# KerkDovan/univer-ocr

Measured on AMD Instinct MI355X. Metric: document-images/sec (fwd+bwd) on 256x512 synthetic pages, higher is better.
Workload: dtype f32; 1 GPU; BASELINE configs[2]: my_model train step (fwd+loss+bwd+L2+SGD) of Monochrome+Paragraph+Line on (32,256,512,1) pages and Char on (32,32,64,1) line strips per GPU; batch_per_gpu=32, global_batch=32, optimizer=sgd, parallelism=dp1, h2d_inclusive=False, input_grads=True, hip_graphs=True, pipelined_lanes=True, hw_queues=4

## Files before the change

univer-ocr_amd/csrc/conv_fast.hip:

```cpp
#include "finish_group.h"
#include "conv_dims.h"

namespace {

template <int C, typename TA>
__device__ __forceinline__ void load_vec(const TA* __restrict__ p, float (&v)[C]) {
    if constexpr (C == 1) {
        v[0] = ld1(p);
    } else if constexpr (C == 2) {
        const float2 t = ld2(p);
        v[0] = t.x;
        v[1] = t.y;
    } else {
        static_assert(C % 4 == 0, "channel count must be 1, 2 or a multiple of 4");
#pragma unroll
        for (int q = 0; q < C / 4; ++q) {
            const float4 t = ld4(p + 4 * q);
            v[4 * q] = t.x;
            v[4 * q + 1] = t.y;
            v[4 * q + 2] = t.z;
            v[4 * q + 3] = t.w;
        }
    }
}
// ... 740 lines not shown
                if constexpr (CIN == 1 && PX % 4 == 0) {
                    constexpr int PWC = KW / 2, OFFS = (4 - PWC % 4) % 4;
                    if (d.pw == PWC && d.w % 4 == 0) {
                        load_row_c1<NXV, OFFS>(xb + (size_t)iyc * d.w, ix0 - OFFS, d.w, row_ok, pad, xv);
                        vec_done = true;
                    }
                }
                if (!vec_done) {
#pragma unroll
                    for (int j = 0; j < NXV; ++j) {
                        const int ix = ix0 + j;
                        if constexpr (CLAMP) {
                            load_vec<CIN>(xb + ((size_t)iyc * d.w + min(max(ix, 0), d.w - 1)) * CIN, xv[j]);
                            if (!(row_ok && ix >= 0 && ix < d.w)) {
#pragma unroll
                                for (int c = 0; c < CIN; ++c) xv[j][c] = pad;
                            }
                        } else {
                            if (row_ok && ix >= 0 && ix < d.w) {
                                load_vec<CIN>(xb + ((size_t)iy * d.w + ix) * CIN, xv[j]);
                            } else {
#pragma unroll
                                for (int c = 0; c < CIN; ++c) xv[j][c] = pad;
                            }
                        }
                    }
                }
#pragma unroll
                for (int kx = 0; kx < KW; ++kx)
#pragma unroll
                    for (int c = 0; c < CIN; ++c)
#pragma unroll
                        for (int o = 0; o < COB; ++o)
#pragma unroll
                            for (int p = 0; p < PX; ++p)
                                acc[((kyl * KW + kx) * CIN + c) * COB + o] += xv[p * SW + kx][c] * g[p][o];
            }
        }
    }
    lane_reduce_scatter<C::NP>(acc, lane);
    int base = 0;
#pragma unroll
    for (int s = 0; s < 6; ++s)
        if (lane & (32 >> s)) base += C::NP >> (s + 1);
#pragma unroll
    for (int r = 0; r < C::NP / 64; ++r) red[wv][base + r] = acc[r];
    __syncthreads();
    const int tid = wv * 64 + lane;
    float* out = partial + ((size_t)blockIdx.y * gridDim.x + blockIdx.x) * C::NP;
    for (int a = tid; a < C::NP; a += 256) out[a] = red[0][a] + red[1][a] + red[2][a] + red[3][a];
}

template <int KH, int KW, int CIN, int COUT, int KYR, int COB, int NW, int NP>
__global__ __launch_bounds__(256) void conv_wgrad_fast_finish(const float* __restrict__ partial, float* __restrict__ dw,
                                                              float* __restrict__ db, int nblocks, int use_bias,
                                                              int accumulate, float unscale) {
    __shared__ double smem[16];
    const int a = blockIdx.x, grp = blockIdx.y;
    constexpr int OCG = COUT / COB;
    const int kyg = grp / OCG, ocg = grp % OCG;
    const float* src = partial + (size_t)grp * nblocks * NP + a;
    double s = 0.0;
    for (int i = threadIdx.x; i < nblocks; i += blockDim.x) s += (double)src[(size_t)i * NP];
    s = block_reduce_sum(s, smem);
    if (threadIdx.x != 0) return;
    float* dst;
    if (a < NW) {
        const int o = a % COB, t = a / COB;
        const int c = t % CIN, tap = t / CIN;
        const int kx = tap % KW, kyl = tap / KW;
        dst = dw + (((size_t)(kyg * KYR + kyl) * KW + kx) * CIN + c) * COUT + ocg * COB + o;
    } else {
        if (kyg != 0) return;
        dst = db + ocg * COB + (a - NW);
        if (!use_bias) s = 0.0;
    }
    s *= (double)unscale;
    *dst = accumulate ? (float)((double)*dst + s) : (float)s;
}

namespace t542 {
constexpr int TH = 16, TW = 64, WH = TH + 4, WW = TW + 4, NW = 40, NB = 2, NACC = NW + NB, NP = 64;
__device__ __forceinline__ int swz(int row, int c) { return row * WW + (c & 3) * (WW / 4) + (c >> 2); }
struct Taprows {
    static constexpr int TH = t542::TH, TW = t542::TW, NW = t542::NW, NB = t542::NB, ROW = NACC;
};
}

template <typename TA>
__global__ __launch_bounds__(320) void conv_wgrad_t542(const TA* __restrict__ x, const TA* __restrict__ dy,
                                                       float* __restrict__ partial, int h, int wd, float pad,
                                                       int tiles_per_block) {
    using namespace t542;
    __shared__ float4 xs[WH * WW];
    __shared__ float2 gs[TH * TW];
    const int tid = threadIdx.x, lane = tid & 63, ky = tid >> 6;
    const int x0 = blockIdx.x * TW, b = blockIdx.z;
    const int tile0 = blockIdx.y * tiles_per_block, tiles_y = (h + TH - 1) / TH;
    const TA* xb = x + (size_t)b * h * wd * 4;
    const TA* gb = dy + (size_t)b * h * wd * 2;
    float acc[NP];
#pragma unroll
    for (int a = 0; a < NP; ++a) acc[a] = 0.f;
    const int cg = lane & 15, rsub = lane >> 4;
    const int t_end = min(tiles_y, tile0 + tiles_per_block);
    for (int t = tile0; t < t_end; ++t) {
        const int y0 = t * TH;
        __syncthreads();
        for (int e = tid; e < WH * WW; e += 320) {
            const int r = e / WW, c = e - r * WW;
            const int gy = y0 - 2 + r, gx = x0 - 2 + c;
            float4 v = ld4(xb + ((size_t)min(max(gy, 0), h - 1) * wd + min(max(gx, 0), wd - 1)) * 4);
            if (gy < 0 || gy >= h || gx < 0 || gx >= wd) v = make_float4(pad, pad, pad, pad);
            xs[swz(r, c)] = v;
        }
        for (int e = tid; e < TH * TW; e += 320) {
            const int r = e / TW, c = e - r * TW;
            const int gy = y0 + r, gx = x0 + c;
            float2 v = ld2(gb + ((size_t)min(gy, h - 1) * wd + min(gx, wd - 1)) * 2);
            if (gy >= h || gx >= wd) v = make_float2(0.f, 0.f);
            gs[e] = v;
        }
        __syncthreads();
#pragma unroll 1
        for (int it = 0; it < TH / 4; ++it) {
            const int r = it * 4 + rsub;
            float g[4][2];
            {
                const float4* gp = reinterpret_cast<const float4*>(gs + r * TW + 4 * cg);
                const float4 g01 = gp[0], g23 = gp[1];
                g[0][0] = g01.x, g[0][1] = g01.y, g[1][0] = g01.z, g[1][1] = g01.w;
                g[2][0] = g23.x, g[2][1] = g23.y, g[3][0] = g23.z, g[3][1] = g23.w;
            }
            float xv[8][4];
#pragma unroll
            for (int j = 0; j < 8; ++j) {
                const float4 v = xs[swz(r + ky, 4 * cg + j)];
                xv[j][0] = v.x, xv[j][1] = v.y, xv[j][2] = v.z, xv[j][3] = v.w;
            }
#pragma unroll
            for (int kx = 0; kx < 5; ++kx)
#pragma unroll
                for (int ci = 0; ci < 4; ++ci)
#pragma unroll
                    for (int co = 0; co < 2; ++co)
#pragma unroll
                        for (int px = 0; px < 4; ++px) acc[(kx * 4 + ci) * 2 + co] += xv[px + kx][ci] * g[px][co];
            if (ky == 0) {
#pragma unroll
                for (int px = 0; px < 4; ++px) {
                    acc[40] += g[px][0];
                    acc[41] += g[px][1];
                }
            }
        }
    }
    lane_reduce_scatter<NP>(acc, lane);
    const size_t blk = ((size_t)blockIdx.z * gridDim.y + blockIdx.y) * gridDim.x + blockIdx.x;
    if (lane < NACC) partial[(blk * 5 + ky) * NACC + lane] = acc[0];
}

template <int CIN, int COUT>
struct S2Cfg {
    static constexpr int TH = 8, TW = 32, WH = 2 * TH + 3, WW = 2 * TW + 3;
    static constexpr int NW = 5 * CIN * COUT, NACC = NW + COUT;
    static constexpr int NP = ((NACC + 63) / 64) * 64;
    static constexpr int NB = COUT, ROW = NP;
};

template <int CIN, int COUT, typename TA>
__global__ __launch_bounds__(320) void conv_wgrad_s2_tiled(const TA* __restrict__ x, const TA* __restrict__ dy,
                                                           float* __restrict__ partial, int h, int wd, int oh, int ow,
                                                           float pad, int tiles_per_block) {
    using C = S2Cfg<CIN, COUT>;
    __shared__ __attribute__((aligned(16))) float xs[C::WH * C::WW * CIN];
    __shared__ float gs[C::TH * C::TW * COUT];
    const int tid = threadIdx.x, lane = tid & 63, ky = tid >> 6;
    const int ox0 = blockIdx.x * C::TW, b = blockIdx.z;
    const int tile0 = blockIdx.y * tiles_per_block, tiles_y = (oh + C::TH - 1) / C::TH;
    const TA* xb = x + (size_t)b * h * wd * CIN;
    const TA* gb = dy + (size_t)b * oh * ow * COUT;
    float acc[C::NP];
#pragma unroll
    for (int a = 0; a < C::NP; ++a) acc[a] = 0.f;
    const int t_end = min(tiles_y, tile0 + tiles_per_block);
    for (int t = tile0; t < t_end; ++t) {
        const int oy0 = t * C::TH;
        __syncthreads();
        if constexpr (sizeof(TA) == 4 && (CIN == 1 || CIN == 4)) {
            using VX = std::conditional_t<CIN == 1, float, float4>;
            stage_batched<C::WH * C::WW, 320, 4, VX>(
                tid,
                [&](int e, bool& inside) {
                    const int r = e / C::WW, c = e - r * C::WW;
                    const int gy = 2 * oy0 - 2 + r, gx = 2 * ox0 - 2 + c;
                    inside = gy >= 0 && gy < h && gx >= 0 && gx < wd;
                    return reinterpret_cast<const VX*>(xb + ((size_t)min(max(gy, 0), h - 1) * wd + min(max(gx, 0), wd - 1)) * CIN);
                },
                [&](int e, VX v, bool inside) {
                    if constexpr (CIN == 1) xs[e] = inside ? v : pad;
                    else *reinterpret_cast<float4*>(xs + e * 4) = inside ? v : make_float4(pad, pad, pad, pad);
                });
        } else {
        for (int e = tid; e < C::WH * C::WW; e += 320) {
            const int r = e / C::WW, c = e - r * C::WW;
            const int gy = 2 * oy0 - 2 + r, gx = 2 * ox0 - 2 + c;
            float v[CIN];
            load_vec<CIN>(xb + ((size_t)min(max(gy, 0), h - 1) * wd + min(max(gx, 0), wd - 1)) * CIN, v);
            const bool in = gy >= 0 && gy < h && gx >= 0 && gx < wd;
#pragma unroll
            for (int ci = 0; ci < CIN; ++ci) xs[e * CIN + ci] = in ? v[ci] : pad;
        }
        }
        for (int e = tid; e < C::TH * C::TW; e += 320) {
            const int r = e / C::TW, c = e - r * C::TW;
            const int gy = oy0 + r, gx = ox0 + c;
            float v[COUT];
            load_vec<COUT>(gb + ((size_t)min(gy, oh - 1) * ow + min(gx, ow - 1)) * COUT, v);
            const bool in = gy < oh && gx < ow;
#pragma unroll
            for (int co = 0; co < COUT; ++co) gs[e * COUT + co] = in ? v[co] : 0.f;
        }
        __syncthreads();
#pragma unroll 1
        for (int it = 0; it < C::TH * C::TW / 64; ++it) {
            const int e = it * 64 + lane, r = e / C::TW, c = e - r * C::TW;
            float g[COUT];
#pragma unroll
            for (int co = 0; co < COUT; ++co) g[co] = gs[e * COUT + co];
            const float* xr = xs + ((2 * r + ky) * C::WW + 2 * c) * CIN;
#pragma unroll
            for (int kx = 0; kx < 5; ++kx)
#pragma unroll
                for (int ci = 0; ci < CIN; ++ci) {
                    const float xv = xr[kx * CIN + ci];
#pragma unroll
                    for (int co = 0; co < COUT; ++co) acc[(kx * CIN + ci) * COUT + co] += xv * g[co];
                }
            if (ky == 0) {
#pragma unroll
                for (int co = 0; co < COUT; ++co) acc[C::NW + co] += g[co];
            }
// ... 213 lines not shown
}

int uocr_conv_dgrad_fast(uocr_ctx* ctx, int dtype, const void* dy, const void* w, void* dx, const ConvDims& d,
                         const ActMask& mask) {
    const bool f32 = UOCR_DTYPE_BASE(dtype) == UOCR_F32;
    const C16Args c16{dy, w, nullptr, dx, 0.f, 0, UOCR_ACT_NONE, 0.f, mask};
    if (f32 && is_c16_same(d, 16, 1))
        return launch_c16(ctx, conv_c16_expand<3, 3, 2, true>, 2, c16, d, 1, UOCR_CONV_C16_EXPAND);
    if (f32 && is_c16_same(d, 1, 16))
        return launch_c16(ctx, conv_c16_reduce<3, 3, 4, true>, 4, c16, d, 1, UOCR_CONV_C16_REDUCE);
    if (f32 && d.kh == 5 && d.kw == 3 && d.sh == 2 && d.sw == 1 && d.ph == 0 && d.pw == 1 && d.cin == 1 && d.cout == 64 &&
        d.h <= 65535 && d.n <= 65535) {
        hipLaunchKernelGGL(conv_dgrad_c64s2, dim3((unsigned)((d.w + 15) / 16), d.h, d.n), dim3(256), 0, ctx->stream,
                           (const float*)dy, (const float*)w, (float*)dx, d.n, d.h, d.w, d.oh, d.ow,
                           (const float*)mask.y, mask.act, (float)mask.alpha);
        UOCR_LAUNCH_CHECK(ctx);
        uocr_note_conv(ctx, 1, UOCR_CONV_DGRAD_C64S2);
        return UOCR_OK;
    }
    if (is_5x5_s2_pad2(d) && ((d.cin == 1 && (d.cout == 1 || d.cout == 4)) || (d.cin == 4 && d.cout == 4))) {
        const dim3 grid(((d.w + 1) / 2 + 63) / 64, ((d.h + 1) / 2 + 3) / 4, d.n), block(64, 4);
        const FastDims fd{d.n, d.h, d.w, d.oh, d.ow, d.ph, d.pw};
        const int rc = uocr_act_tags<1>(ctx, UOCR_ACT_NONE, mask.act, [&](auto kinds) -> int {
            using K = decltype(kinds);
            using D = ActKinds<UOCR_ACT_DYN, UOCR_ACT_DYN>;
            UOCR_DISPATCH_TA(ctx, dtype, {
                auto launch = [&](auto kernel) {
                    hipLaunchKernelGGL(kernel, grid, block, 0, ctx->stream, (const TA*)dy, (const float*)w, (TA*)dx, fd,
                                       (const TA*)mask.y, mask.act, (float)mask.alpha);
                };
                if (d.cin == 4) launch(conv_dgrad_s2<4, 4, TA, K>);
                else if (d.cout == 1) launch(conv_dgrad_s2<1, 1, TA, D>);
                else launch(conv_dgrad_s2<1, 4, TA, D>);
            });
            UOCR_LAUNCH_CHECK(ctx);
            return UOCR_OK;
        });
        if (rc != UOCR_OK) return rc;
        uocr_note_conv(ctx, 1, UOCR_CONV_DGRAD_S2);
        return UOCR_OK;
    }
    int rc = UOCR_OK;
    if (with_fast_conv(d, [&](auto fc) { rc = uocr_noted_conv(ctx, 1, fc.DX_KERNEL, fc.dgrad(ctx, dtype, dy, w, dx, d, mask)); }))
        return rc;
    UOCR_FAIL(ctx, UOCR_ERR_UNSUPPORTED, "no fast conv kernel for this shape");
}

int uocr_conv_wgrad_fast(uocr_ctx* ctx, int dtype, const void* x, const void* dy, void* dw, void* db,
                         const ConvDims& d, double pad_value, int use_bias, int accumulate) {
    const bool f32 = UOCR_DTYPE_BASE(dtype) == UOCR_F32;
    if (f32 && is_c16_same(d, 16, 1) && pad_value == 0.0) {
        constexpr int NA = 3 * 3 * 4 + 1;
        const long budget = uocr_budget(ctx, 2048);
        int rows = (int)((d.n * d.h + budget - 1) / budget);
        rows = ((rows + 3) / 4) * 4;
        if (rows > d.h) rows = ((d.h + 3) / 4) * 4;
        const int nbands = (d.h + rows - 1) / rows, nblocks = nbands * d.n;
        uocr_note_split(ctx, nblocks, (long long)((d.h + 3) / 4) * d.n);
        int rc = uocr_need_workspace(ctx, (size_t)nblocks * 4 * NA * sizeof(float));
        if (rc) return rc;
        float* partial = (float*)ctx->workspace;
        hipLaunchKernelGGL((conv_c16_wgrad<3, 3>), dim3(nblocks), dim3(64, 4), 0, ctx->stream, (const float*)x,
                           (const float*)dy, partial, d.h, d.w, d.ph, d.pw, rows, nbands);
        UOCR_LAUNCH_CHECK(ctx);
        hipLaunchKernelGGL((conv_c16_wgrad_finish<3, 3>), dim3(NA, 4), dim3(256), 0, ctx->stream,
                           (const float*)partial, (float*)dw, (float*)db, nblocks, use_bias, accumulate);
        UOCR_LAUNCH_CHECK(ctx);
        uocr_note_conv(ctx, 2, UOCR_CONV_C16_WGRAD);
        return UOCR_OK;
    }
    if (is_5x5_s2_pad2(d) && ctx->opt_tiled == 1 && d.cin == 1 && d.cout == 4)
        return launch_wgrad_taprows<S2Cfg<1, 4>>(
            ctx, dtype, UOCR_CONV_WGRAD_S2_TILED, d.n, d.oh, d.ow, dw, db, use_bias, accumulate,
            [&](auto ta, dim3 grid, float* partial, int per_block) {
                using TA = decltype(ta);
                hipLaunchKernelGGL((conv_wgrad_s2_tiled<1, 4, TA>), grid, dim3(320), 0, ctx->stream, (const TA*)x,
                                   (const TA*)dy, partial, d.h, d.w, d.oh, d.ow, (float)pad_value, per_block);
            });
    if (is_5x5_s1_pad2(d) && d.cin == 4 && d.cout == 2)
        return launch_wgrad_taprows<t542::Taprows>(
            ctx, dtype, UOCR_CONV_WGRAD_T542, d.n, d.h, d.w, dw, db, use_bias, accumulate,
            [&](auto ta, dim3 grid, float* partial, int per_block) {
                using TA = decltype(ta);
                hipLaunchKernelGGL((conv_wgrad_t542<TA>), grid, dim3(320), 0, ctx->stream, (const TA*)x, (const TA*)dy,
                                   partial, d.h, d.w, (float)pad_value, per_block);
            });
    int rc = UOCR_OK;
    if (with_fast_conv(d, [&](auto fc) {
            rc = uocr_noted_conv(ctx, 2, UOCR_CONV_TABLE_FAST, fc.wgrad(ctx, dtype, x, dy, dw, db, d, pad_value, use_bias, accumulate));
        }))
        return rc;
    UOCR_FAIL(ctx, UOCR_ERR_UNSUPPORTED, "no fast conv kernel for this shape");
}
```

univer-ocr_amd/csrc/ctx.hip:

```cpp
#include <cstdlib>

#include "finish_group.h"
#include "gemm.h"
#include "uocr_common.h"

extern "C" {

int uocr_abi_version(void) { return UOCR_ABI_VERSION; }

int uocr_ctx_create(int device, size_t workspace_bytes, uocr_ctx** out) {
    if (!out || device < 0) return UOCR_ERR_ARG;
    *out = nullptr;
    int count = 0;
    if (hipGetDeviceCount(&count) != hipSuccess || device >= count) return UOCR_ERR_HIP;
    if (hipSetDevice(device) != hipSuccess) return UOCR_ERR_HIP;
    uocr_ctx* ctx = new uocr_ctx();
    ctx->device = device;
#ifdef UOCR_EXPERIMENTS
    if (const char* e = getenv("UOCR_H3")) ctx->opt_h3 = atoi(e);
#endif
    if (const char* e = getenv("UOCR_PAIR_PF")) ctx->opt_pair_pf = atoi(e);
    if (const char* e = getenv("UOCR_WGRAD_BANDS")) ctx->opt_wgrad_bands = atoi(e);
    if (hipStreamCreateWithFlags(&ctx->stream, hipStreamNonBlocking) != hipSuccess) {
        delete ctx;
// ... 8 lines not shown
            return UOCR_ERR_HIP;
        }
        ctx->workspace_bytes = workspace_bytes;
    }
    if (hipMalloc((void**)&ctx->sync, UOCR_SYNC_WORDS * sizeof(unsigned)) != hipSuccess ||
        hipMemsetAsync(ctx->sync, 0, UOCR_SYNC_WORDS * sizeof(unsigned), ctx->stream) != hipSuccess ||
        hipStreamSynchronize(ctx->stream) != hipSuccess) {
        if (ctx->sync) hipFree(ctx->sync);
        if (ctx->workspace) hipFree(ctx->workspace);
        hipStreamDestroy(ctx->stream);
        delete ctx;
        return UOCR_ERR_HIP;
    }
    *out = ctx;
    return UOCR_OK;
}

int uocr_ctx_create_cu_mask(int device, size_t workspace_bytes, const uint32_t* cu_mask, int mask_words, uocr_ctx** out) {
    if (!out || !cu_mask || mask_words <= 0) return UOCR_ERR_ARG;
    int rc = uocr_ctx_create(device, workspace_bytes, out);
    if (rc != UOCR_OK) return rc;
    uocr_ctx* ctx = *out;
    hipStream_t masked = nullptr;
    if (hipExtStreamCreateWithCUMask(&masked, (uint32_t)mask_words, cu_mask) != hipSuccess) {
        uocr_ctx_destroy(ctx);
        *out = nullptr;
        return UOCR_ERR_HIP;
    }
    hipStreamDestroy(ctx->stream);
    ctx->stream = masked;
    int cus = 0;
    for (int i = 0; i < mask_words; ++i) cus += __builtin_popcount(cu_mask[i]);
    if (cus > 0 && cus < ctx->cu_count) ctx->cu_count = cus;
    return UOCR_OK;
}

int uocr_ctx_destroy(uocr_ctx* ctx) {
    UOCR_CHECK_CTX(ctx);
    hipSetDevice(ctx->device);
    hipStreamSynchronize(ctx->stream);
    if (ctx->workspace) hipFree(ctx->workspace);
    if (ctx->sync) hipFree(ctx->sync);
    uocr_gemm_defer_free(ctx);
    uocr_finish_defer_free(ctx);
    if (ctx->owns_stream) hipStreamDestroy(ctx->stream);
    delete ctx;
    return UOCR_OK;
}

int uocr_ctx_set_stream(uocr_ctx* ctx, void* hip_stream) {
    UOCR_CHECK_CTX(ctx);
    if (ctx->owns_stream) {
        UOCR_HIP(ctx, hipStreamSynchronize(ctx->stream));
        UOCR_HIP(ctx, hipStreamDestroy(ctx->stream));
        ctx->owns_stream = false;
    }
    ctx->stream = (hipStream_t)hip_stream;
    return UOCR_OK;
}

int uocr_ctx_set_option(uocr_ctx* ctx, const char* key, int value) {
    UOCR_CHECK_CTX(ctx);
    UOCR_REQUIRE(ctx, key != nullptr);
    if (!strcmp(key, "mfma")) ctx->opt_mfma = value;
    else if (!strcmp(key, "fast_paths")) ctx->opt_fast = value;
    else if (!strcmp(key, "tiled")) ctx->opt_tiled = value;
    else if (!strcmp(key, "split_blocks")) ctx->opt_split = value;
    else if (!strcmp(key, "split_min")) ctx->opt_split_min = value;
    else if (!strcmp(key, "gemm_bm")) ctx->opt_bm = value;
    else if (!strcmp(key, "xcd_remap")) ctx->opt_xcd = value;
    else if (!strcmp(key, "h16")) ctx->opt_h16 = value;
    else if (!strcmp(key, "t32")) {
        if (value & ~UOCR_T32_BUILT)
            UOCR_FAIL(ctx, UOCR_ERR_UNSUPPORTED, "option t32 = %d asks for kernels this library was built without "
                      "(UOCR_BUILD_EXPERIMENTS=1 ./build.sh)", value);
        ctx->opt_t32 = value;
    }
    else if (!strcmp(key, "pair_band")) ctx->opt_pair_band = value;
    else if (!strcmp(key, "pair_g")) ctx->opt_pair_g = value;
    else if (!strcmp(key, "group_blocks")) ctx->opt_group_blocks = value;
    else if (!strcmp(key, "wgrad_bands") && value >= 0) ctx->opt_wgrad_bands = value;
    else if (!strcmp(key, "max_blocks") && value >= 0) ctx->opt_max_blocks = value;
    else if (!strcmp(key, "act_dispatch")) ctx->opt_act_dispatch = value != 0;
    else if (!strcmp(key, "h3")) {
#ifndef UOCR_EXPERIMENTS
        if (value) UOCR_FAIL(ctx, UOCR_ERR_UNSUPPORTED, "option h3: this library was built without conv_h3 "
                             "(UOCR_BUILD_EXPERIMENTS=1 ./build.sh)");
#endif
        ctx->opt_h3 = value;
    }
    else if (!strcmp(key, "pair_pf")) ctx->opt_pair_pf = value;
    else UOCR_FAIL(ctx, UOCR_ERR_ARG, "unknown option '%s'", key);
    return UOCR_OK;
}

int uocr_ctx_last_split(uocr_ctx* ctx, int* blocks, long long* items) {
    return uocr_report_read(ctx, UOCR_REPORT_SPLIT, blocks, items);
}

int uocr_ctx_last_gemm(uocr_ctx* ctx, int* bm, int* gm, int* gn, int* nsplit) {
    return uocr_report_read(ctx, UOCR_REPORT_GEMM, bm, gm, gn, nsplit);
}

int uocr_ctx_last_gemm_group(uocr_ctx* ctx, int* problems, int* split_problems) {
    return uocr_report_read(ctx, UOCR_REPORT_GEMM_GROUP, problems, split_problems);
}

int uocr_ctx_last_pair(uocr_ctx* ctx, int* kernel, int* g, int* mode, int* pf, int* nw, int* blocks_x, int* bands,
                       int* band_h) {
    return uocr_report_read(ctx, UOCR_REPORT_PAIR, kernel, g, mode, pf, nw, blocks_x, bands, band_h);
}

int uocr_ctx_last_conv(uocr_ctx* ctx, int* entry, int* kernel) {
    return uocr_report_read(ctx, UOCR_REPORT_CONV, entry, kernel);
}

void* uocr_ctx_get_stream(uocr_ctx* ctx) { return ctx ? (void*)ctx->stream : nullptr; }

int uocr_ctx_reserve_workspace(uocr_ctx* ctx, size_t bytes) {
    UOCR_CHECK_CTX(ctx);
    if (bytes <= ctx->workspace_bytes) return UOCR_OK;
    UOCR_HIP(ctx, hipSetDevice(ctx->device));
    UOCR_HIP(ctx, hipStreamSynchronize(ctx->stream));
    if (ctx->workspace) UOCR_HIP(ctx, hipFree(ctx->workspace));
    ctx->workspace = nullptr;
    ctx->workspace_bytes = 0;
    UOCR_HIP(ctx, hipMalloc(&ctx->workspace, bytes));
    ctx->workspace_bytes = bytes;
    return UOCR_OK;
}

const char* uocr_last_error(uocr_ctx* ctx) { return ctx ? ctx->err : "null context"; }

int uocr_malloc(uocr_ctx* ctx, size_t bytes, void** out) {
    UOCR_CHECK_CTX(ctx);
    UOCR_REQUIRE(ctx, out != nullptr);
    UOCR_HIP(ctx, hipSetDevice(ctx->device));
    UOCR_HIP(ctx, hipMalloc(out, bytes ? bytes : 1));
    return UOCR_OK;
}

int uocr_free(uocr_ctx* ctx, void* ptr) {
    UOCR_CHECK_CTX(ctx);
    if (ptr) UOCR_HIP(ctx, hipFree(ptr));
    return UOCR_OK;
}

int uocr_memset_zero(uocr_ctx* ctx, void* ptr, size_t bytes) {
    UOCR_CHECK_CTX(ctx);
    if (!bytes) return UOCR_OK;
    UOCR_REQUIRE(ctx, ptr != nullptr);
    UOCR_HIP(ctx, hipMemsetAsync(ptr, 0, bytes, ctx->stream));
    return UOCR_OK;
}

int uocr_h2d(uocr_ctx* ctx, void* dst, const void* src_host, size_t bytes) {
    UOCR_CHECK_CTX(ctx);
    if (!bytes) return UOCR_OK;
    UOCR_REQUIRE(ctx, dst && src_host);
    UOCR_HIP(ctx, hipMemcpyAsync(dst, src_host, bytes, hipMemcpyHostToDevice, ctx->stream));
    return UOCR_OK;
}

int uocr_d2h_sync(uocr_ctx* ctx, void* dst_host, const void* src, size_t bytes) {
    UOCR_CHECK_CTX(ctx);
    if (!bytes) return UOCR_OK;
// ... 106 lines not shown
```

univer-ocr_amd/csrc/uocr_common.h:

```cpp
#pragma once
#include <hip/hip_runtime.h>
#include <stdint.h>
#include <stdio.h>
#include <string.h>

#include <type_traits>

#include "univer_hip.h"

enum uocr_report_id {
    UOCR_REPORT_SPLIT,
    UOCR_REPORT_GEMM,
    UOCR_REPORT_GEMM_GROUP,
    UOCR_REPORT_PAIR,
    UOCR_REPORT_CONV,
    UOCR_REPORT_LABEL,
    UOCR_REPORT_LABEL_BATCH,
    UOCR_REPORT_CHAR_LABEL,
    UOCR_REPORT_LINE_CROP,
    UOCR_REPORT_ROTATE,
    UOCR_REPORT_ROTATION_SEARCH,
    UOCR_REPORT_PRED_TO_TEXT,
    UOCR_REPORT_PACK_LINES,
    UOCR_REPORT_COUNT
};
constexpr int UOCR_REPORT_VALUES = 8;

struct uocr_ctx {
    int device = 0;
    hipStream_t stream = nullptr;
    bool owns_stream = true;
    void* workspace = nullptr;
    size_t workspace_bytes = 0;
    const double* snap_src = nullptr;
    int snap_count = 0;
    double* snap_ring = nullptr;
    int snap_ring_len = 0;
    unsigned* snap_counter = nullptr;
    void* gemm_defer = nullptr;
    void* finish_defer = nullptr;
    unsigned* sync = nullptr;
    int cu_count = 256;
    int opt_mfma = 1;
    int opt_fast = 1;
    int opt_tiled = 1;
    int opt_split = 1024;
    int opt_split_min = 3;
    int opt_xcd = 1;
    int opt_bm = 0;
    int opt_h16 = 1;
    int opt_t32 = 2;
    int opt_pair_band = 0;
    int opt_pair_pf = -1;
    int opt_h3 = 0;
    int opt_group_blocks = 0;
    int opt_wgrad_bands = 0;
    int opt_pair_g = 4;
    int opt_act_dispatch = 1;
    int opt_max_blocks = 0;
    long long report[UOCR_REPORT_COUNT][UOCR_REPORT_VALUES] = {};
    char err[512] = {};
};

constexpr int UOCR_SYNC_WORDS = 1 << 18;
#ifdef UOCR_EXPERIMENTS
constexpr int UOCR_T32_BUILT = 255;
#else
constexpr int UOCR_T32_BUILT = 2;
#endif

#define UOCR_FAIL(ctx, code, ...)                                   \
    do {                                                            \
        if (ctx) snprintf((ctx)->err, sizeof((ctx)->err), __VA_ARGS__); \
        return (code);                                              \
    } while (0)

#define UOCR_HIP(ctx, call)                                                              \
    do {                                                                                 \
        hipError_t e_ = (call);                                                          \
        if (e_ != hipSuccess)                                                            \
            UOCR_FAIL(ctx, UOCR_ERR_HIP, "%s failed: %s (%s:%d)", #call, hipGetErrorString(e_), \
                      __FILE__, __LINE__);                                               \
    } while (0)

#define UOCR_LAUNCH_CHECK(ctx)                                                           \
    do {                                                                                 \
        hipError_t e_ = hipGetLastError();                                               \
        if (e_ != hipSuccess)                                                            \
            UOCR_FAIL(ctx, UOCR_ERR_HIP, "kernel launch failed: %s (%s:%d)", hipGetErrorString(e_), \
                      __FILE__, __LINE__);                                               \
    } while (0)

#define UOCR_REQUIRE(ctx, cond)                                                          \
    do {                                                                                 \
        if (!(cond)) UOCR_FAIL(ctx, UOCR_ERR_ARG, "bad argument: %s (%s:%d)", #cond, __FILE__, __LINE__); \
    } while (0)

#define UOCR_CHECK_CTX(ctx) \
    do {                    \
        if (!(ctx)) return UOCR_ERR_ARG; \
    } while (0)

template <typename... V>
static inline void uocr_note(uocr_ctx* ctx, uocr_report_id id, V... v) {
    static_assert(sizeof...(V) >= 1 && sizeof...(V) <= UOCR_REPORT_VALUES, "a report holds 1 to UOCR_REPORT_VALUES values");
    long long* slot = ctx->report[id];
    ((*slot++ = (long long)v), ...);
}
template <typename... T>
static inline int uocr_report_read(uocr_ctx* ctx, uocr_report_id id, T*... out) {
    static_assert(sizeof...(T) >= 1 && sizeof...(T) <= UOCR_REPORT_VALUES, "a report holds 1 to UOCR_REPORT_VALUES values");
    UOCR_CHECK_CTX(ctx);
    if (!(out && ...)) UOCR_FAIL(ctx, UOCR_ERR_ARG, "bad argument: null out pointer of launch report %d", (int)id);
    const long long* slot = ctx->report[id];
    ((*out = (T)*slot++), ...);
    return UOCR_OK;
}

#define UOCR_DISPATCH(ctx, dtype, ...)                                   \
    do {                                                                 \
        if ((dtype) == UOCR_F32) { using T = float; __VA_ARGS__; }       \
        else if ((dtype) == UOCR_F64) { using T = double; __VA_ARGS__; } \
        else UOCR_FAIL(ctx, UOCR_ERR_DTYPE, "unknown dtype %d", (int)(dtype)); \
    } while (0)

#define UOCR_DISPATCH_ACT(ctx, dtype, ...)                                                        \
    do {                                                                                          \
        const int base_ = UOCR_DTYPE_BASE(dtype);                                                 \
        if (base_ == UOCR_F32) { using TS = float; using T = float; __VA_ARGS__; }                \
        else if (base_ == UOCR_F64) { using TS = double; using T = double; __VA_ARGS__; }         \
        else if (base_ == UOCR_F16) { using TS = _Float16; using T = float; __VA_ARGS__; }        \
        else UOCR_FAIL(ctx, UOCR_ERR_DTYPE, "unknown dtype %d", (int)(dtype));                    \
    } while (0)

#define UOCR_DISPATCH_STORAGE(ctx, dtype, ...)                                                    \
    do {                                                                                          \
        const int base_ = UOCR_DTYPE_BASE(dtype);                                                 \
        if (base_ == UOCR_F32) { using T = float; __VA_ARGS__; }                                  \
        else if (base_ == UOCR_F64) { using T = double; __VA_ARGS__; }                            \
        else if (base_ == UOCR_F16) { using T = _Float16; __VA_ARGS__; }                          \
        else UOCR_FAIL(ctx, UOCR_ERR_DTYPE, "unknown dtype %d", (int)(dtype));                    \
// ... 171 lines not shown
__device__ __forceinline__ void st4(_Float16* p, float4 v) {
    uocr_h4 h;
    h.x = (_Float16)v.x;
    h.y = (_Float16)v.y;
    h.z = (_Float16)v.z;
    h.w = (_Float16)v.w;
    *reinterpret_cast<uocr_h4*>(p) = h;
}

#define UOCR_DISPATCH_TA(ctx, dtype, ...)                                                          \
    do {                                                                                           \
        const int base_ = UOCR_DTYPE_BASE(dtype);                                                  \
        if (base_ == UOCR_F32) { using TA = float; __VA_ARGS__; }                                  \
        else if (base_ == UOCR_F16) { using TA = _Float16; __VA_ARGS__; }                          \
        else UOCR_FAIL(ctx, UOCR_ERR_DTYPE, "dtype %d: this kernel exists for float32 / float16 only", (int)(dtype)); \
    } while (0)

static inline bool uocr_aligned_act(const void* p, int dtype) {
    return (reinterpret_cast<uintptr_t>(p) & (UOCR_DTYPE_BASE(dtype) == UOCR_F16 ? 7u : 15u)) == 0;
}
static inline bool uocr_aligned16(const void* p) { return (reinterpret_cast<uintptr_t>(p) & 15u) == 0; }

__device__ __forceinline__ float act_apply(float v, int act, float alpha) {
    switch (act) {
        case UOCR_ACT_RELU: return v * (v >= 0.f ? 1.f : 0.f);
        case UOCR_ACT_LEAKY: return v * ((v >= 0.f ? 1.f : 0.f) + alpha * (v < 0.f ? 1.f : 0.f));
        case UOCR_ACT_SIGMOID: return 1.f / (1.f + expf(-v));
        default: return v;
    }
}

template <typename T>
__device__ __forceinline__ T act_grad_from_output(T y, int act, T alpha) {
    if (act == UOCR_ACT_LEAKY) return y >= T(0) ? T(1) : alpha;
    if (act == UOCR_ACT_SIGMOID) return y * (T(1) - y);
    return T(1);
}

constexpr int UOCR_ACT_DYN = -1;
template <int ACT, int MASK>
struct ActKinds {
    static constexpr int act = ACT, mask = MASK;
    static constexpr bool dynamic = ACT == UOCR_ACT_DYN;
};
template <bool KEEP, class K>
using ActKindsIf = std::conditional_t<KEEP, K, ActKinds<UOCR_ACT_DYN, UOCR_ACT_DYN>>;
template <int KIND>
__host__ __device__ __forceinline__ int act_kind(int argument) {
    return KIND == UOCR_ACT_DYN ? argument : KIND;
}
template <int SIDE, class F>
static inline int uocr_act_tags(const uocr_ctx* ctx, int act, int mask_act, F&& f) {
    if (ctx->opt_act_dispatch) {
        if constexpr (SIDE == 0) {
            if (mask_act == UOCR_ACT_NONE && act == UOCR_ACT_NONE) return f(ActKinds<UOCR_ACT_NONE, UOCR_ACT_NONE>{});
            if (mask_act == UOCR_ACT_NONE && act == UOCR_ACT_LEAKY) return f(ActKinds<UOCR_ACT_LEAKY, UOCR_ACT_NONE>{});
            if (mask_act == UOCR_ACT_NONE && act == UOCR_ACT_SIGMOID) return f(ActKinds<UOCR_ACT_SIGMOID, UOCR_ACT_NONE>{});
        } else {
            if (act == UOCR_ACT_NONE && mask_act == UOCR_ACT_NONE) return f(ActKinds<UOCR_ACT_NONE, UOCR_ACT_NONE>{});
            if (act == UOCR_ACT_NONE && mask_act == UOCR_ACT_LEAKY) return f(ActKinds<UOCR_ACT_NONE, UOCR_ACT_LEAKY>{});
        }
    }
    return f(ActKinds<UOCR_ACT_DYN, UOCR_ACT_DYN>{});
}

template <int COUNT, int NT, int BATCH, typename V, typename Addr, typename Put>
__device__ __forceinline__ void stage_batched(int tid, Addr addr, Put put) {
    constexpr int K = (COUNT + NT - 1) / NT;
#pragma unroll
    for (int k0 = 0; k0 < K; k0 += BATCH) {
        V v[BATCH];
        bool in[BATCH];
#pragma unroll
        for (int k = 0; k < BATCH; ++k)
            if (k0 + k < K) v[k] = *addr(min(tid + NT * (k0 + k), COUNT - 1), in[k]);
#pragma unroll
        for (int k = 0; k < BATCH; ++k)
            if (k0 + k < K) {
                const int i = tid + NT * (k0 + k);
                if (i < COUNT) put(i, v[k], in[k]);
            }
    }
}

struct TileWalk {
    int strip, trow, img;
    int qx, qy, qz;
    __device__ __forceinline__ TileWalk(int first, int step, int tiles_x, int tiles_y) {
        strip = first % tiles_x;
        int r = first / tiles_x;
        trow = r % tiles_y;
        img = r / tiles_y;
        qx = step % tiles_x;
        r = step / tiles_x;
        qy = r % tiles_y;
        qz = r / tiles_y;
    }
    __device__ __forceinline__ void next(int tiles_x, int tiles_y) {
        strip += qx;
        int carry = strip >= tiles_x;
        strip -= carry ? tiles_x : 0;
        trow += qy + carry;
        carry = trow >= tiles_y;
        trow -= carry ? tiles_y : 0;
        img += qz + carry;
    }
};

int uocr_finish_sum(uocr_ctx* ctx, const double* partial, int count, double scale, double* out, int accumulate);
```

Before: 34110 images/s.

## Add dedicated loader waves with double-buffered stages to t542 wgrad kernel

Adds two producer waves to the 5x5 stride-1 4->2 weight-gradient kernel. They stage 8-row slices of input and output-gradient into double-buffered shared memory while the five compute waves consume the previous slice. This is meant to hide global load latency behind the FMA trips instead of stalling all waves on the load-then-compute barrier. The cost is more threads per block, twice the shared-memory footprint, and a barrier per half tile, which may reduce occupancy. A new option enables the path by default, and the old single-buffer path is kept.

```diff
diff --git a/univer-ocr_amd/csrc/conv_fast.hip b/univer-ocr_amd/csrc/conv_fast.hip
--- a/univer-ocr_amd/csrc/conv_fast.hip
+++ b/univer-ocr_amd/csrc/conv_fast.hip
@@ -846,82 +846,174 @@
 namespace t542 {
 constexpr int TH = 16, TW = 64, WH = TH + 4, WW = TW + 4, NW = 40, NB = 2, NACC = NW + NB, NP = 64;
 __device__ __forceinline__ int swz(int row, int c) { return row * WW + (c & 3) * (WW / 4) + (c >> 2); }
+constexpr int LOADER_SR = 8, LOADER_WAVES = 2;
 struct Taprows {
     static constexpr int TH = t542::TH, TW = t542::TW, NW = t542::NW, NB = t542::NB, ROW = NACC;
 };
-}
-
-template <typename TA>
-__global__ __launch_bounds__(320) void conv_wgrad_t542(const TA* __restrict__ x, const TA* __restrict__ dy,
-                                                       float* __restrict__ partial, int h, int wd, float pad,
-                                                       int tiles_per_block) {
+template <int SR, int L>
+struct Stage {
+    static_assert(TH % SR == 0 && SR % 4 == 0, "a stage is a whole number of trips, a tile a whole number of stages");
+    static constexpr int NT = 64 * (L > 0 ? L : 1), PER_TILE = TH / SR, ROWS = SR + 4;
+    static constexpr int MAIN = ROWS * TW, SIDE = (ROWS * 4 + NT - 1) / NT * NT, GCOUNT = SR * TW;
+    static constexpr int XIMG = ROWS * WW, NBUF = L > 0 ? 2 : 1;
+    static_assert(L == 0 || (MAIN % NT == 0 && GCOUNT % NT == 0), "whole rows per loader wave");
+    static_assert(NBUF * (XIMG * 16 + GCOUNT * 8) <= 65536, "static shared memory");
+};
+__device__ __forceinline__ float4 widen(float4 v) { return v; }
+__device__ __forceinline__ float2 widen(float2 v) { return v; }
+__device__ __forceinline__ float4 widen(uocr_h4 v) { return make_float4((float)v.x, (float)v.y, (float)v.z, (float)v.w); }
+__device__ __forceinline__ float2 widen(uocr_h2 v) { return make_float2((float)v.x, (float)v.y); }
+
+template <int ROWS>
+__device__ __forceinline__ void trips(const float4* __restrict__ xs, const float2* __restrict__ gs, int ky, int lane,
+                                      float (&acc)[NP]) {
+    const int cg = lane & 15, rsub = lane >> 4;
+#pragma unroll 1
+    for (int it = 0; it < ROWS / 4; ++it) {
+        const int r = it * 4 + rsub;
+        float g[4][2];
+        {
+            const float4* gp = reinterpret_cast<const float4*>(gs + r * TW + 4 * cg);
+            const float4 g01 = gp[0], g23 = gp[1];
+            g[0][0] = g01.x, g[0][1] = g01.y, g[1][0] = g01.z, g[1][1] = g01.w;
+            g[2][0] = g23.x, g[2][1] = g23.y, g[3][0] = g23.z, g[3][1] = g23.w;
+        }
+        float xv[8][4];
+        const float4* xp = xs + swz(r + ky, 4 * cg);
+#pragma unroll
+        for (int j = 0; j < 8; ++j) {
+            const float4 v = xp[(j & 3) * (WW / 4) + (j >> 2)];
+            xv[j][0] = v.x, xv[j][1] = v.y, xv[j][2] = v.z, xv[j][3] = v.w;
+        }
+#pragma unroll
+        for (int kx = 0; kx < 5; ++kx)
+#pragma unroll
+            for (int ci = 0; ci < 4; ++ci)
+#pragma unroll
+                for (int co = 0; co < 2; ++co)
+#pragma unroll
+                    for (int px = 0; px < 4; ++px) acc[(kx * 4 + ci) * 2 + co] += xv[px + kx][ci] * g[px][co];
+        if (ky == 0) {
+#pragma unroll
+            for (int px = 0; px < 4; ++px) {
+                acc[40] += g[px][0];
+                acc[41] += g[px][1];
+            }
+        }
+    }
+}
+}
+
+template <typename TA, int SR, int L>
+__global__ __launch_bounds__(320 + 64 * L) void conv_wgrad_t542(const TA* __restrict__ x, const TA* __restrict__ dy,
+                                                                float* __restrict__ partial, int h, int wd, float pad,
+                                                                int tiles_per_block) {
     using namespace t542;
-    __shared__ float4 xs[WH * WW];
-    __shared__ float2 gs[TH * TW];
-    const int tid = threadIdx.x, lane = tid & 63, ky = tid >> 6;
+    using S = Stage<SR, L>;
+    __shared__ float4 xs[S::NBUF * S::XIMG];
+    __shared__ float2 gs[S::NBUF * S::GCOUNT];
+    const int tid = threadIdx.x, lane = tid & 63;
+    const int wave = __builtin_amdgcn_readfirstlane(tid >> 6);
     const int x0 = blockIdx.x * TW, b = blockIdx.z;
     const int tile0 = blockIdx.y * tiles_per_block, tiles_y = (h + TH - 1) / TH;
     const TA* xb = x + (size_t)b * h * wd * 4;
     const TA* gb = dy + (size_t)b * h * wd * 2;
-    float acc[NP];
-#pragma unroll
-    for (int a = 0; a < NP; ++a) acc[a] = 0.f;
-    const int cg = lane & 15, rsub = lane >> 4;
     const int t_end = min(tiles_y, tile0 + tiles_per_block);
-    for (int t = tile0; t < t_end; ++t) {
-        const int y0 = t * TH;
+    const size_t blk = ((size_t)blockIdx.z * gridDim.y + blockIdx.y) * gridDim.x + blockIdx.x;
+    if constexpr (L == 0) {
+        float acc[NP];
+#pragma unroll
+        for (int a = 0; a < NP; ++a) acc[a] = 0.f;
+        for (int t = tile0; t < t_end; ++t) {
+            const int y0 = t * TH;
+            __syncthreads();
+            for (int e = tid; e < WH * WW; e += 320) {
+                const int r = e / WW, c = e - r * WW;
+                const int gy = y0 - 2 + r, gx = x0 - 2 + c;
+                float4 v = ld4(xb + ((size_t)min(max(gy, 0), h - 1) * wd + min(max(gx, 0), wd - 1)) * 4);
+                if (gy < 0 || gy >= h || gx < 0 || gx >= wd) v = make_float4(pad, pad, pad, pad);
+                xs[swz(r, c)] = v;
+            }
+            for (int e = tid; e < TH * TW; e += 320) {
+                const int r = e / TW, c = e - r * TW;
+                const int gy = y0 + r, gx = x0 + c;
+                float2 v = ld2(gb + ((size_t)min(gy, h - 1) * wd + min(gx, wd - 1)) * 2);
+                if (gy >= h || gx >= wd) v = make_float2(0.f, 0.f);
+                gs[e] = v;
+            }
+            __syncthreads();
+            trips<TH>(xs, gs, wave, lane, acc);
+        }
+        lane_reduce_scatter<NP>(acc, lane);
+        if (lane < NACC) partial[(blk * 5 + wave) * NACC + lane] = acc[0];
+    } else {
+        using VX = std::conditional_t<sizeof(TA) == 4, float4, uocr_h4>;
+        using VG = std::conditional_t<sizeof(TA) == 4, float2, uocr_h2>;
+        const int nstages = (t_end - tile0) * S::PER_TILE;
+        const bool loader = wave >= 5;
+        const int lt = (wave - 5) * 64 + lane;
+        struct Loads {
+            StageRegs<S::MAIN, S::NT, VX> main;
+            StageRegs<S::SIDE, S::NT, VX> side;
+            StageRegs<S::GCOUNT, S::NT, VG> g;
+        };
+        auto row = [](int e) { return __builtin_amdgcn_readfirstlane(e >> 6); };
+        auto top = [&](int s) { return (tile0 + s / S::PER_TILE) * TH + (s % S::PER_TILE) * SR; };
+        auto request = [&](Loads& q, int s) {
+            const int y0 = top(s);
+            auto xsrc = [&](int r, int c) {
+                const int gy = min(max(y0 - 2 + r, 0), h - 1), gx = min(max(x0 - 2 + c, 0), wd - 1);
+                return reinterpret_cast<const VX*>(xb + ((size_t)gy * wd + gx) * 4);
+            };
+            q.main.request(lt, [&](int e) { return xsrc(row(e), e & 63); });
+            q.side.request(lt, [&](int e) { return xsrc(min(e >> 2, S::ROWS - 1), TW + (e & 3)); });
+            q.g.request(lt, [&](int e) {
+                const int r = row(e), c = e & 63;
+                return reinterpret_cast<const VG*>(gb + ((size_t)min(y0 + r, h - 1) * wd + min(x0 + c, wd - 1)) * 2);
+            });
+        };
+        auto commit = [&](const Loads& q, int s) {
+            const int y0 = top(s);
+            float4* xd = xs + (s & 1) * S::XIMG;
+            float2* gd = gs + (s & 1) * S::GCOUNT;
+            auto xput = [&](int r, int c, VX v) {
+                const bool in = ((unsigned)(y0 - 2 + r) < (unsigned)h) & ((unsigned)(x0 - 2 + c) < (unsigned)wd);
+                xd[swz(r, c)] = in ? widen(v) : make_float4(pad, pad, pad, pad);
+            };
+            q.main.commit(lt, [&](int e, VX v) { xput(row(e), e & 63, v); });
+            q.side.commit(lt, [&](int e, VX v) { xput(min(e >> 2, S::ROWS - 1), TW + (e & 3), v); });
+            q.g.commit(lt, [&](int e, VG v) {
+                const bool in = (y0 + row(e) < h) & (x0 + (e & 63) < wd);
+                gd[e] = in ? widen(v) : make_float2(0.f, 0.f);
+            });
+        };
+        auto stage = [&](int s) {
+            Loads q;
+            request(q, s);
+            __builtin_amdgcn_sched_barrier(0);
+            commit(q, s);
+        };
+        if (loader) stage(0);
         __syncthreads();
-        for (int e = tid; e < WH * WW; e += 320) {
-            const int r = e / WW, c = e - r * WW;
-            const int gy = y0 - 2 + r, gx = x0 - 2 + c;
-            float4 v = ld4(xb + ((size_t)min(max(gy, 0), h - 1) * wd + min(max(gx, 0), wd - 1)) * 4);
-            if (gy < 0 || gy >= h || gx < 0 || gx >= wd) v = make_float4(pad, pad, pad, pad);
-            xs[swz(r, c)] = v;
-        }
-        for (int e = tid; e < TH * TW; e += 320) {
-            const int r = e / TW, c = e - r * TW;
-            const int gy = y0 + r, gx = x0 + c;
-            float2 v = ld2(gb + ((size_t)min(gy, h - 1) * wd + min(gx, wd - 1)) * 2);
-            if (gy >= h || gx >= wd) v = make_float2(0.f, 0.f);
-            gs[e] = v;
-        }
-        __syncthreads();
+        if (loader) {
 #pragma unroll 1
-        for (int it = 0; it < TH / 4; ++it) {
-            const int r = it * 4 + rsub;
-            float g[4][2];
-            {
-                const float4* gp = reinterpret_cast<const float4*>(gs + r * TW + 4 * cg);
-                const float4 g01 = gp[0], g23 = gp[1];
-                g[0][0] = g01.x, g[0][1] = g01.y, g[1][0] = g01.z, g[1][1] = g01.w;
-                g[2][0] = g23.x, g[2][1] = g23.y, g[3][0] = g23.z, g[3][1] = g23.w;
-            }
-            float xv[8][4];
-#pragma unroll
-            for (int j = 0; j < 8; ++j) {
-                const float4 v = xs[swz(r + ky, 4 * cg + j)];
-                xv[j][0] = v.x, xv[j][1] = v.y, xv[j][2] = v.z, xv[j][3] = v.w;
-            }
-#pragma unroll
-            for (int kx = 0; kx < 5; ++kx)
-#pragma unroll
-                for (int ci = 0; ci < 4; ++ci)
-#pragma unroll
-                    for (int co = 0; co < 2; ++co)
-#pragma unroll
-                        for (int px = 0; px < 4; ++px) acc[(kx * 4 + ci) * 2 + co] += xv[px + kx][ci] * g[px][co];
-            if (ky == 0) {
-#pragma unroll
-                for (int px = 0; px < 4; ++px) {
-                    acc[40] += g[px][0];
-                    acc[41] += g[px][1];
-                }
-            }
-        }
-    }
-    lane_reduce_scatter<NP>(acc, lane);
-    const size_t blk = ((size_t)blockIdx.z * gridDim.y + blockIdx.y) * gridDim.x + blockIdx.x;
-    if (lane < NACC) partial[(blk * 5 + ky) * NACC + lane] = acc[0];
+            for (int s = 0; s < nstages; ++s) {
+                if (s + 1 < nstages) stage(s + 1);
+                __syncthreads();
+            }
+        } else {
+            float acc[NP];
+#pragma unroll
+            for (int a = 0; a < NP; ++a) acc[a] = 0.f;
+#pragma unroll 1
+            for (int s = 0; s < nstages; ++s) {
+                trips<SR>(xs + (s & 1) * S::XIMG, gs + (s & 1) * S::GCOUNT, wave, lane, acc);
+                __syncthreads();
+            }
+            lane_reduce_scatter<NP>(acc, lane);
+            if (lane < NACC) partial[(blk * 5 + wave) * NACC + lane] = acc[0];
+        }
+    }
 }
 
 template <int CIN, int COUT>
@@ -1301,8 +1393,13 @@
             ctx, dtype, UOCR_CONV_WGRAD_T542, d.n, d.h, d.w, dw, db, use_bias, accumulate,
             [&](auto ta, dim3 grid, float* partial, int per_block) {
                 using TA = decltype(ta);
-                hipLaunchKernelGGL((conv_wgrad_t542<TA>), grid, dim3(320), 0, ctx->stream, (const TA*)x, (const TA*)dy,
-                                   partial, d.h, d.w, (float)pad_value, per_block);
+                auto launch = [&](auto sr, auto l) {
+                    hipLaunchKernelGGL((conv_wgrad_t542<TA, sr(), l()>), grid, dim3(320 + 64 * l()), 0, ctx->stream, (const TA*)x,
+                                       (const TA*)dy, partial, d.h, d.w, (float)pad_value, per_block);
+                };
+                using std::integral_constant;
+                if (ctx->opt_wgrad_loader) launch(integral_constant<int, t542::LOADER_SR>{}, integral_constant<int, t542::LOADER_WAVES>{});
+                else launch(integral_constant<int, t542::TH>{}, integral_constant<int, 0>{});
             });
     int rc = UOCR_OK;
     if (with_fast_conv(d, [&](auto fc) {
diff --git a/univer-ocr_amd/csrc/ctx.hip b/univer-ocr_amd/csrc/ctx.hip
--- a/univer-ocr_amd/csrc/ctx.hip
+++ b/univer-ocr_amd/csrc/ctx.hip
@@ -114,6 +114,7 @@
     else if (!strcmp(key, "wgrad_bands") && value >= 0) ctx->opt_wgrad_bands = value;
     else if (!strcmp(key, "max_blocks") && value >= 0) ctx->opt_max_blocks = value;
     else if (!strcmp(key, "act_dispatch")) ctx->opt_act_dispatch = value != 0;
+    else if (!strcmp(key, "wgrad_loader")) ctx->opt_wgrad_loader = value != 0;
     else if (!strcmp(key, "h3")) {
 #ifndef UOCR_EXPERIMENTS
         if (value) UOCR_FAIL(ctx, UOCR_ERR_UNSUPPORTED, "option h3: this library was built without conv_h3 "
diff --git a/univer-ocr_amd/csrc/uocr_common.h b/univer-ocr_amd/csrc/uocr_common.h
--- a/univer-ocr_amd/csrc/uocr_common.h
+++ b/univer-ocr_amd/csrc/uocr_common.h
@@ -57,6 +57,7 @@
     int opt_wgrad_bands = 0;
     int opt_pair_g = 4;
     int opt_act_dispatch = 1;
+    int opt_wgrad_loader = 1;
     int opt_max_blocks = 0;
     long long report[UOCR_REPORT_COUNT][UOCR_REPORT_VALUES] = {};
     char err[512] = {};
@@ -394,6 +395,23 @@
             }
     }
 }
+
+template <int COUNT, int NT, typename V>
+struct StageRegs {
+    static_assert(COUNT % NT == 0, "pad the staged image to a multiple of the staging threads");
+    static constexpr int K = COUNT / NT;
+    V v[K];
+    template <typename Addr>
+    __device__ __forceinline__ void request(int tid, Addr addr) {
+#pragma unroll
+        for (int k = 0; k < K; ++k) v[k] = *addr(tid + NT * k);
+    }
+    template <typename Put>
+    __device__ __forceinline__ void commit(int tid, Put put) const {
+#pragma unroll
+        for (int k = 0; k < K; ++k) put(tid + NT * k, v[k]);
+    }
+};
 
 struct TileWalk {
     int strip, trow, img;
```

Measured after the change: 34680 images/s, median of 4. +1.7%, better.
